# SoraSuegami/halo2-rsa

Measured on AMD Instinct MI355X. Metric: RSA-2048 pkcs1v15 witness assigns/sec, higher is better.
Workload: dtype u64

## Files before the change

halo2_rsa_amd/csrc/h2r_api.hip:

```cpp
#include <hip/hip_runtime.h>
#include <hip/hip_ext.h>
#include <dlfcn.h>
#include <rccl/rccl.h>

#include <algorithm>
#include <chrono>
#include <cstdio>
#include <cstdlib>
#include <cstring>
#include <functional>
#include <map>
#include <memory>
#include <mutex>
#include <new>
#include <vector>

#include "h2r.h"
#include "h2r_internal.hpp"
#include "h2r_varrows.hpp"
#include "h2r_copymap.hpp"
#include "h2r_layout.hpp"
#include "h2r_lookup.hpp"
#include "h2r_lookup_product.hpp"
#include "h2r_permutation_product.hpp"
#include "h2r_ntt.hpp"
#include "h2r_quotient.hpp"
#include "h2r_open.hpp"
#include "h2r_msm.hpp"
#include "h2r_curve_ntt.hpp"
#include "h2r_transcript.hpp"
#include "h2r_random.hpp"
#include "h2r_verify.hpp"
#include "h2r_muled.hpp"
#include "h2r_rowprog.hpp"
#include "h2r_sha256.hpp"
#include "h2r_check.hpp"
#include "h2r_arena_match.hpp"
#include "h2r_stage_args.hpp"

using namespace h2r;

namespace {

thread_local char g_hip_err[256] = "";

bool hip_ok(hipError_t e, const char *what) {
    if (e == hipSuccess) return true;
    std::snprintf(g_hip_err, sizeof g_hip_err, "%s: %s", what, hipGetErrorString(e));
    return false;
}
#define H2R_CATCH_STATUS catch (const std::bad_alloc &) { return H2R_E_NOMEM; } catch (...) { return H2R_E_INTERNAL; }
#define H2R_CATCH_ZERO catch (...) { return 0; }
#define H2R_CATCH_VOID catch (...) { }
#define H2R_CATCH_STR catch (...) { return ""; }
#define HIP_TRY(expr)                                   \
    do {                                                \
        if (!hip_ok((expr), #expr)) return H2R_E_HIP;   \
    } while (0)

struct DeviceGuard {
    int prev = -1; bool switched = false; hipError_t err = hipSuccess;
    explicit DeviceGuard(int dev) {
        err = hipGetDevice(&prev);
        if (err == hipSuccess && prev != dev) { err = hipSetDevice(dev); switched = err == hipSuccess; }
    }
    ~DeviceGuard() { if (switched) (void)hipSetDevice(prev); }
    DeviceGuard(const DeviceGuard &) = delete;
    DeviceGuard &operator=(const DeviceGuard &) = delete;
};
#define H2R_ON_DEVICE(dev_)                                     \
    DeviceGuard h2r_device_guard_(dev_);                        \
    if (!hip_ok(h2r_device_guard_.err, "hipSetDevice")) return H2R_E_HIP

struct ProfRec { u32 kernel; hipEvent_t a, b; };
std::mutex g_prof_mu;
std::vector<ProfRec> g_prof;
u32 g_prof_cap = 0;
u32 g_prof_gen = 0;
struct ProfScope {
    hipStream_t st; hipEvent_t a = nullptr, b = nullptr; u32 kernel; bool on = false, ext;
    ProfScope(u32 k, hipStream_t s, bool ext_ = false) : st(s), kernel(k), ext(ext_) {
        std::lock_guard<std::mutex> lk(g_prof_mu);
        if (g_prof_cap && g_prof.size() < g_prof_cap && hipEventCreate(&a) == hipSuccess) {
            if (hipEventCreate(&b) != hipSuccess) { (void)hipEventDestroy(a); a = nullptr; return; }
            on = true;
            if (!ext) (void)hipEventRecord(a, st);
        }
    }
    ~ProfScope() {
        if (!on) return;
        if (!ext) (void)hipEventRecord(b, st);
        std::lock_guard<std::mutex> lk(g_prof_mu);
        g_prof.push_back(ProfRec{kernel, a, b});
    }
};
template <class Fn> int32_t stage_launch(u32 kernel_class, hipStream_t st, Fn &&fn) {
    ProfScope ps(kernel_class, st, true);
    HIP_TRY(fn(ps.a, ps.on ? ps.b : nullptr));
    return H2R_OK;
}


inline u64 odd_stride_256(u64 bytes) {
    u64 u = round_up(bytes, 256) / 256;
    u |= 1;
    const u64 r = u % 256;
    if (r >= 24 && r <= 62) u += 65 - r;
    return u * 256;
}

struct DoneRef {
    hipEvent_t ev = nullptr; u32 gen = 0; bool borrowed = false;
    bool alive() const {
        if (!borrowed) return true;
        std::lock_guard<std::mutex> lk(g_prof_mu);
        return gen == g_prof_gen;
    }
};

struct Workspace {
    u64 off_pre;
    u64 off_n;
    u64 off_state;
    u64 total;
};
Workspace workspace_plan(u32 limb_bytes, u32 L, u64 batch, u32 T) {
    Workspace w;
    const u64 arr = round_up(batch * T * (u64)L * limb_bytes, 256);
    w.off_pre = 4 * arr;
    w.off_n = w.off_pre + round_up(4ull * chain_pre_words(128), 256);
    w.off_state = w.off_n + round_up(batch * (u64)L * limb_bytes, 256);
    w.total = w.off_state + round_up(2 * batch * (u64)L * limb_bytes, 256) + 256;
    return w;
}

}

struct h2r_ctx {
    h2r_params params;
    h2r_layout layout;
    u32 L, K;
    U256 word_max;
    u8 *const_rec_dev;
    u32 *advice_desc_dev = nullptr;
    u32 cells_nwv = 1;
    u64 *cells_ktab_dev = nullptr;
    std::vector<u8> const_rec_host;
    u32 tab0_len, tab1_off, tab1_len, tab2_off, tab2_len, hist_len;
    u8 refresh_inc[2 * 128 + 8]; u32 refresh_nf;
    u64 field_p[4];
    FieldConsts fc;
    h2r_advice_repr repr;
    MontK mk;
    MontK *mk_dev = nullptr;
    u32 num_cus, lds_per_cu;
    mutable std::mutex pipe_mu;
    mutable h2r_pipeline *pipe = nullptr;
    mutable std::mutex side_mu;
    mutable hipStream_t side_stream = nullptr;
    mutable hipEvent_t side_fork = nullptr, side_join = nullptr;
    struct RowProg { std::vector<RpRow> host; RpRow *dev = nullptr; std::vector<u32> inv_rows; u32 *inv_dev = nullptr; };
    mutable std::mutex prog_mu;
    mutable std::map<u32, RowProg> progs;
    mutable std::mutex check_mu;
    mutable std::map<std::vector<u8>, CheckKind *> check_tabs;
};

namespace {

void put_le(u8 *dst, const U256 &v, u32 nbytes) { std::memcpy(dst, v.v, nbytes); }

void build_const_record(h2r_ctx *c) {
    const h2r_layout &lo = c->layout;
    c->const_rec_host.assign(lo.record_stride, 0);
    u8 *r = c->const_rec_host.data();
    const u32 w = lo.limb_width, C = lo.num_cols;
    U256 acc_extra;
    for (u32 i = 0; i < C; ++i) {
        acc_extra = acc_extra + c->word_max;
        U256 q_acc = acc_extra.shr(w);
        u64 mod_acc = acc_extra.low(w);
// ... 2076 lines not shown
    return lookup_hist_values_impl(ctx, cfg, values, value_bytes, values_per_elem, num_elems, values_per_elem * value_bytes, value_bytes,
                                   bit_len, sublimb_bits, nullptr, hist, stream);
} H2R_CATCH_STATUS

int32_t h2r_lookup_hist_values_strided(const h2r_ctx *ctx, const h2r_lookup_config *cfg, const void *values, uint32_t value_bytes,
                                       uint64_t values_per_elem, uint64_t num_elems, uint64_t elem_stride, uint64_t value_stride,
                                       uint32_t bit_len, uint32_t sublimb_bits, const uint8_t *status, uint32_t *hist,
                                       h2r_stream_t stream) try {
    return lookup_hist_values_impl(ctx, cfg, values, value_bytes, values_per_elem, num_elems, elem_stride, value_stride, bit_len,
                                   sublimb_bits, status, hist, stream);
} H2R_CATCH_STATUS

extern "C++" {
namespace {
template <typename F>
void fresh_range_runs(const AuxGeom &g, u32 op, F &&run) {
    u64 off = 0;
    const u32 L = g.L;
    auto add = [&](u32 n) { run(off + 2 * g.SB, n, g.STEP); run(off + 2 * g.SB + g.RA, n, g.STEP); off += g.add_sz(n); };
    auto eq = [&](u32 n) { off += g.eq_sz(n); };
    auto subu = [&](u32 n1) { run(off, n1, g.RA); off += g.cl_sz(n1); add(n1); eq(n1 + 1); };
    auto sub = [&](u32 nA, u32 nB) {
        const u32 m = nA > nB ? nA : nB, n1 = m + 1;
        add(m); subu(n1);
        off += 16; off += AuxGeom::a16((u64)n1 * g.LB); off += AuxGeom::a16((u64)m * g.LB);
        subu(n1);
    };
    auto lt = [&]() { sub(L, L); eq(L); off += 16; };
    switch (op) {
        case FRESH_ADD: add(L); break;
        case FRESH_SUB: case FRESH_IS_LESS_THAN_OR_EQUAL: case FRESH_IS_GREATER_THAN: sub(L, L); break;
        case FRESH_ADD_MOD: add(L); sub(L + 1, L); break;
        case FRESH_SUB_MOD: sub(L, L); sub(L, L + 1); break;
        case FRESH_IS_LESS_THAN: case FRESH_IS_IN_FIELD: case FRESH_IS_GREATER_THAN_OR_EQUAL: lt(); break;
        default: break;
    }
}
int32_t lookup_hist_fresh_impl(const h2r_ctx *ctx, const h2r_lookup_config *cfg, uint32_t op, const void *trace, uint64_t first_off,
                               uint64_t elem_stride, uint64_t num_elems, const uint8_t *status, uint32_t *hist, h2r_stream_t stream) {
    if (!ctx || !cfg || !trace || !hist) return H2R_E_NULL;
    if (ctx->params.device < 0 || op >= FRESH_OP_COUNT) return H2R_E_UNSUPPORTED;
    if (cfg->n_rows == 0 || cfg->n_rows > (u32)LOOKUP_MAX_ROWS) return H2R_E_SHAPE;
    const h2r_layout &lo = ctx->layout;
    LookupFreshArgs a;
    std::memset(&a, 0, sizeof a);
    a.status = status;
    const int32_t rc = range_shape(*cfg, lo.limb_width, lo.limb_sub_bits, &a.limb);
    if (rc) return rc;
    const AuxGeom g(ctx->L, lo.limb_width);
    bool too_many = false;
    fresh_range_runs(g, op, [&](u64 off, u32 n, u32 stride) {
        if (a.n_runs >= 16) { too_many = true; return; }
        a.run_off[a.n_runs] = (u32)off; a.run_n[a.n_runs] = n; a.run_stride[a.n_runs] = stride; ++a.n_runs;
    });
    if (too_many) return H2R_E_UNSUPPORTED;
    if (num_elems == 0 || a.n_runs == 0) return H2R_OK;
    a.trace = static_cast<const u8 *>(trace); a.first_off = first_off; a.elem_stride = elem_stride; a.num_elems = num_elems;
    a.sub_off = lo.limb_bytes; a.n_rows = cfg->n_rows; a.hist = hist;
    H2R_ON_DEVICE(ctx->params.device);
    hipStream_t st = static_cast<hipStream_t>(stream);
    ProfScope ps(H2R_KERNEL_HIST, st);
    HIP_TRY(launch_lookup_hist_fresh(a, st));
    return H2R_OK;
}
}
}

int32_t h2r_lookup_hist_verify(const h2r_ctx *ctx, const h2r_lookup_config *cfg, const h2r_verify_layout *vl, const void *trace,
                               uint64_t num_elems, const uint8_t *status, uint32_t *hist, h2r_stream_t stream) try {
    if (!ctx || !cfg || !vl || !trace || !hist) return H2R_E_NULL;
    if (vl->pow.off_records == UINT64_MAX) return H2R_E_SHAPE;
    int32_t rc = lookup_hist_fresh_impl(ctx, cfg, H2R_OP_IS_IN_FIELD, trace, vl->off_in_field, vl->elem_stride, num_elems, status, hist, stream);
    if (!rc) rc = h2r_lookup_hist_records(ctx, cfg, trace, vl->pow.off_records, vl->elem_stride, num_elems, vl->pow.num_mul_mods, status, hist, stream);
    if (!rc) rc = lookup_hist_values_impl(ctx, cfg, static_cast<const u8 *>(trace) + vl->off_em + 12, 4, 2, num_elems, vl->elem_stride, 12, 32, 4,
                                          status, hist, stream);
    return rc;
} H2R_CATCH_STATUS

int32_t h2r_lookup_hist_fresh_op(const h2r_ctx *ctx, const h2r_lookup_config *cfg, uint32_t op, const void *trace, uint64_t first_off,
                                 uint64_t elem_stride, uint64_t num_elems, uint32_t *hist, h2r_stream_t stream) try {
    return lookup_hist_fresh_impl(ctx, cfg, op, trace, first_off, elem_stride, num_elems, nullptr, hist, stream);
} H2R_CATCH_STATUS

uint64_t h2r_lookup_workspace_bytes(const h2r_lookup_config *cfg, uint64_t num_elems) try {
    if (!cfg || cfg->n_rows == 0 || cfg->n_rows > (u32)LOOKUP_MAX_ROWS) return 0;
    return num_elems * LOOKUP_ARGS * lookup_slot_bytes(cfg->n_rows) + 256;
} H2R_CATCH_ZERO

int32_t h2r_lookup_permuted_columns(const h2r_ctx *ctx, const h2r_lookup_config *cfg, const uint32_t *hist, const uint64_t *theta,
                                    uint64_t num_elems, uint32_t usable_rows, uint32_t arg_mask, void *a_perm_out,
                                    void *s_perm_out, uint64_t out_elem_stride, uint8_t *status, void *workspace,
                                    h2r_stream_t stream) try {
    if (!ctx || !cfg || !hist || !theta || !a_perm_out || !s_perm_out || !workspace) return H2R_E_NULL;
    if (ctx->params.device < 0) return H2R_E_UNSUPPORTED;
    if (cfg->n_rows == 0 || cfg->n_rows > (u32)LOOKUP_MAX_ROWS || cfg->n_lens == 0 || cfg->n_lens > H2R_LOOKUP_MAX_LENS) return H2R_E_SHAPE;
    if (usable_rows < cfg->n_rows || out_elem_stride < (u64)LOOKUP_ARGS * usable_rows * 32 || (out_elem_stride & 15) ||
        (reinterpret_cast<u64>(a_perm_out) & 15) || (reinterpret_cast<u64>(s_perm_out) & 15)) return H2R_E_SHAPE;
    if (num_elems == 0 || !(arg_mask & 31u)) return H2R_OK;
    if (num_elems * LOOKUP_ARGS >= (1ull << 31) || num_elems > 65535) return H2R_E_UNSUPPORTED;
    H2R_ON_DEVICE(ctx->params.device);
    hipStream_t st = static_cast<hipStream_t>(stream);
    u8 *ws = reinterpret_cast<u8 *>(round_up(reinterpret_cast<u64>(workspace), 256));
    if (status) HIP_TRY(hipMemsetAsync(status, 0, num_elems, st));
    LookupSetupArgs sa;
    std::memset(&sa, 0, sizeof sa);
    sa.hist = hist; sa.theta = theta; sa.num_elems = num_elems; sa.usable_rows = usable_rows; sa.n_rows = cfg->n_rows;
    sa.n_lens = cfg->n_lens; sa.arg_mask = arg_mask & 31u;
    for (u32 i = 0; i < cfg->n_lens; ++i) { sa.tag[i] = cfg->tag[i]; sa.row_off[i] = cfg->row_off[i]; sa.bit_len[i] = cfg->bit_len[i]; }
    sa.f = ctx->fc; sa.ws = ws; sa.status = status;
    sa.mont = (ctx->repr.flags & H2R_ADVICE_MONTGOMERY) ? 1u : 0u;
    HIP_TRY(launch_lookup_setup(sa, st));
    LookupFillArgs fa;
    std::memset(&fa, 0, sizeof fa);
    fa.ws = ws; fa.num_elems = num_elems; fa.usable_rows = usable_rows; fa.n_rows = cfg->n_rows; fa.arg_mask = arg_mask & 31u;
    fa.rows_per_block = 256; fa.round_robin = 0; fa.status = status;
#ifdef H2R_DEV_KNOBS
    if ((arg_mask >> 8) & 0xffu) fa.rows_per_block = 256u * ((arg_mask >> 8) & 0xffu);
    fa.round_robin = (arg_mask >> 16) & 1u;
#endif
    fa.a_perm = static_cast<u8 *>(a_perm_out); fa.s_perm = static_cast<u8 *>(s_perm_out); fa.out_elem_stride = out_elem_stride;
    return stage_launch(H2R_KERNEL_LOOKUP, st, [&](hipEvent_t a, hipEvent_t b) { return launch_lookup_fill(fa, st, a, b); });
} H2R_CATCH_STATUS

int32_t h2r_field_eval(const h2r_ctx *ctx, uint32_t op, const uint64_t a[4], const uint64_t b[4], uint64_t out[4]) try {
    if (!ctx || !a || !out || (op < 3 && !b)) return H2R_E_NULL;
    Fe x, y = fe_zero(), r;
    for (int k = 0; k < 4; ++k) { x.v[k] = a[k]; if (b) y.v[k] = b[k]; }
    if (ge_p(x.v, ctx->fc.p) || (op < 3 && ge_p(y.v, ctx->fc.p))) return H2R_E_SHAPE;
    switch (op) {
        case 0: r = fe_add(x, y, ctx->fc.p); break;
        case 1: r = fe_sub(x, y, ctx->fc.p); break;
        case 2: r = fe_mul(x, y, ctx->fc); break;
        case 3: if (fe_is_zero(x)) return H2R_E_SHAPE; r = fe_inv(x, ctx->fc); break;
        case 4: if (fe_is_zero(x)) return H2R_E_SHAPE; r = fe_inv_fermat(x, ctx->fc); break;
        case 5: if (fe_is_zero(x)) return H2R_E_SHAPE; r = fe_inv_fast(x, ctx->fc); break;
        case 6: {
            u32 d[8], t[8]; int K = 1;
            for (int k = 0; k < 4; ++k) { d[2 * k] = (u32)x.v[k]; d[2 * k + 1] = (u32)(x.v[k] >> 32); }
            for (int k = 0; k < 8; ++k) if (d[k]) K = k + 1;
            switch (K) {
                case 1: { const u32 q[1] = {d[0]}; mont_short<1>(q, ctx->mk.bk[1], ctx->mk.p, ctx->mk.n0inv, t); break; }
                case 2: { const u32 q[2] = {d[0], d[1]}; mont_short<2>(q, ctx->mk.bk[2], ctx->mk.p, ctx->mk.n0inv, t); break; }
                case 3: { const u32 q[3] = {d[0], d[1], d[2]}; mont_short<3>(q, ctx->mk.bk[3], ctx->mk.p, ctx->mk.n0inv, t); break; }
                case 4: { const u32 q[4] = {d[0], d[1], d[2], d[3]}; mont_short<4>(q, ctx->mk.bk[4], ctx->mk.p, ctx->mk.n0inv, t); break; }
                case 5: { const u32 q[5] = {d[0], d[1], d[2], d[3], d[4]}; mont_short<5>(q, ctx->mk.bk[5], ctx->mk.p, ctx->mk.n0inv, t); break; }
                case 6: { const u32 q[6] = {d[0], d[1], d[2], d[3], d[4], d[5]}; mont_short<6>(q, ctx->mk.bk[6], ctx->mk.p, ctx->mk.n0inv, t); break; }
                case 7: { const u32 q[7] = {d[0], d[1], d[2], d[3], d[4], d[5], d[6]}; mont_short<7>(q, ctx->mk.bk[7], ctx->mk.p, ctx->mk.n0inv, t); break; }
                default: mont_short<8>(d, ctx->mk.bk[8], ctx->mk.p, ctx->mk.n0inv, t); break;
            }
            for (int k = 0; k < 4; ++k) r.v[k] = ((u64)t[2 * k + 1] << 32) | t[2 * k];
            break;
        }
        case 7: r = fe_from_mont(x, ctx->fc); break;
        case 8: r = fe_to_mont(x, ctx->fc); break;
        case 9: {
            u32 d[8], t[8]; int bits = 1;
            for (int k = 0; k < 4; ++k) { d[2 * k] = (u32)x.v[k]; d[2 * k + 1] = (u32)(x.v[k] >> 32); }
            for (int k = 0; k < 256; ++k) if ((d[k / 32] >> (k % 32)) & 1u) bits = k + 1;
            switch ((bits + 29) / 30) {
                case 1: mont_bits<30, 8>(d, ctx->mk, t); break;
                case 2: mont_bits<60, 8>(d, ctx->mk, t); break;
                case 3: mont_bits<90, 8>(d, ctx->mk, t); break;
                case 4: mont_bits<120, 8>(d, ctx->mk, t); break;
                case 5: mont_bits<150, 8>(d, ctx->mk, t); break;
                case 6: mont_bits<180, 8>(d, ctx->mk, t); break;
                case 7: mont_bits<210, 8>(d, ctx->mk, t); break;
                case 8: mont_bits<240, 8>(d, ctx->mk, t); break;
                default: mont_bits<256, 8>(d, ctx->mk, t); break;
            }
            for (int k = 0; k < 4; ++k) r.v[k] = ((u64)t[2 * k + 1] << 32) | t[2 * k];
            break;
        }
        default: return H2R_E_UNSUPPORTED;
    }
    for (int k = 0; k < 4; ++k) out[k] = r.v[k];
    return H2R_OK;
} H2R_CATCH_STATUS

namespace {
struct Out { u8 *p; };
inline void emit(Out &o, const u8 *src, u32 n) { std::memcpy(o.p, src, n); o.p += n; }
inline void emit_wide(Out &o, const h2r_layout &lo, const u8 *rec, int pl_lo, u64 idx) {
    emit(o, rec + lo.plane_off[pl_lo] + idx * 16, lo.wide_bytes < 16 ? lo.wide_bytes : 16);
    if (lo.wide_bytes > 16) emit(o, rec + lo.plane_off[pl_lo + 1] + idx * 8, lo.wide_bytes - 16);
}
inline void emit_acc(Out &o, const h2r_layout &lo, const u8 *rec, int pl_lo, u32 j, u32 im) {
    const u64 g = j / lo.acc_steps_per_group, st = j % lo.acc_steps_per_group;
    emit(o, rec + lo.plane_off[pl_lo] + g * lo.acc_lo_group_bytes + st * lo.acc_lo_row_bytes + (u64)im * 16, lo.wide_bytes < 16 ? lo.wide_bytes : 16);
    if (lo.wide_bytes > 16) emit(o, rec + lo.plane_off[pl_lo + 1] + (u64)(j >> 1) * lo.acc_hi_group_bytes + (u64)im * 16 + (j & 1) * 8, lo.wide_bytes - 16);
}
inline void emit_plane(Out &o, const h2r_layout &lo, const u8 *rec, int pl, u64 idx, u32 n) {
    emit(o, rec + lo.plane_off[pl] + idx * lo.plane_elem[pl], n);
}
}

static u8 *flatten_parts(const h2r_layout &lo, const u8 *rec, u8 *outp, u32 parts, const u64 *fp = nullptr) {
    const u32 L = lo.num_limbs, C = lo.num_cols;
    Out o{outp};
    if (parts & 1)
        for (int which = 0; which < 2; ++which)
            for (u32 k = 0; k < L; ++k) {
                emit_plane(o, lo, rec, which ? H2R_PL_R : H2R_PL_Q, k, lo.limb_bytes);
                emit_plane(o, lo, rec, which ? H2R_PL_R_SUB : H2R_PL_Q_SUB, k, lo.limb_nsub);
            }
// ... 459 lines not shown
int32_t fresh_row_prog(const h2r_ctx *ctx, uint32_t op, uint32_t flags, const h2r_ctx::RowProg **out) {
    if (op >= FRESH_OP_COUNT) return H2R_E_UNSUPPORTED;
    const bool assert_one = (flags & H2R_ADVICE_ASSERT_ONE) != 0;
    return row_prog(ctx, op | (assert_one ? 256u : 0u), [&](RowProgBuilder &rb) { return rb.build(op, assert_one); }, out);
}
int32_t launch_row_prog(const h2r_ctx *ctx, const h2r_ctx::RowProg *rp, RowProgArgs &ra, hipStream_t st) {
    ra.prog = rp->dev; ra.rows = (u32)rp->host.size(); ra.f = ctx->fc; ra.mk = ctx->mk_dev;
    ra.inv_rows = rp->inv_dev; ra.n_inv = (u32)rp->inv_rows.size();
    const long sr_k = knobs().rowprog_stage_rows;
    const u32 sr_env = (sr_k == 64 || sr_k == 128 || sr_k == 256) ? (u32)sr_k : 0u;
    const u32 sr = sr_env ? sr_env : ((ctx->repr.flags & H2R_ADVICE_MONTGOMERY) ? 64u : 256u);
    const u64 blocks = ra.batch * ((ra.rows + sr - 1) / sr);
    if (blocks == 0) return H2R_OK;
    if (blocks >= (1ull << 31)) return H2R_E_UNSUPPORTED;
    const u32 w = ctx->layout.limb_width;
    if (const int32_t rc = stage_launch(H2R_KERNEL_EMIT, st, [&](hipEvent_t a, hipEvent_t b) { return launch_rowprog_shape(w, sr, ra, (u32)blocks, st, a, b); })) return rc;
    if (ra.n_inv) {
        const u32 nt = sr == 64 ? 64u : 256u;
        const u64 ib = (ra.batch * ra.n_inv + nt - 1) / nt;
        if (ib >= (1ull << 31)) return H2R_E_UNSUPPORTED;
        HIP_TRY(launch_rowprog_inv_shape(w, nt, ra, (u32)ib, st));
    }
    return H2R_OK;
}
}

uint32_t h2r_fresh_op_advice_rows(const h2r_ctx *ctx, uint32_t op, uint32_t flags) try {
    const h2r_ctx::RowProg *rp = nullptr;
    if (!ctx || fresh_row_prog(ctx, op, flags, &rp)) return 0;
    return (uint32_t)rp->host.size();
} H2R_CATCH_ZERO

int32_t h2r_fresh_op_row_kinds(const h2r_ctx *ctx, uint32_t op, uint32_t flags, uint8_t *kinds_out) try {
    if (!ctx || !kinds_out) return H2R_E_NULL;
    const h2r_ctx::RowProg *rp = nullptr;
    const int32_t rc = fresh_row_prog(ctx, op, flags, &rp);
    if (rc) return rc;
    for (size_t r = 0; r < rp->host.size(); ++r) kinds_out[r] = (uint8_t)rp->host[r].kind;
    return H2R_OK;
} H2R_CATCH_STATUS

namespace {
int32_t fresh_emit_advice(const h2r_ctx *ctx, uint32_t op, uint32_t flags, const void *a, const void *b, const void *n,
                          const void *trace, uint64_t first_off, uint64_t elem_stride, uint64_t batch, const uint8_t *status,
                          const AdviceDst *dst_in, void *advice_out, uint64_t out_stride, h2r_stream_t stream) {
    if (!ctx || !a || !trace || (!dst_in && !advice_out)) return H2R_E_NULL;
    if (ctx->params.device < 0) return H2R_E_UNSUPPORTED;
    const h2r_ctx::RowProg *rp = nullptr;
    int32_t rc = fresh_row_prog(ctx, op, flags, &rp);
    if (rc) return rc;
    const bool needs_b = op != FRESH_IS_ZERO, needs_n = op == FRESH_ADD_MOD || op == FRESH_SUB_MOD;
    if ((needs_b && !b) || (needs_n && !n)) return H2R_E_NULL;
    u64 es = 0;
    rc = h2r_fresh_op_layout(ctx, op, &es, nullptr, nullptr);
    if (rc) return rc;
    if (elem_stride == 0) elem_stride = es;
    const u64 rows = rp->host.size();
    if ((first_off & 15) || (elem_stride & 15)) return H2R_E_SHAPE;
    AdviceDst dst;
    if (dst_in) dst = *dst_in;
    else if ((rc = advice_dst(ctx, advice_out, out_stride, rows, batch, &dst))) return rc;
    if (batch == 0) return H2R_OK;
    RowProgArgs ra;
    std::memset(&ra, 0, sizeof ra);
    ra.a = a; ra.b = b ? b : a; ra.n = n ? n : a;
    ra.a_stride = ctx->L;
    ra.n_stride = (flags & H2R_F_SHARED_MODULUS) ? 0 : ctx->L;
    ra.b_stride = (!needs_n && (flags & H2R_F_SHARED_MODULUS)) ? 0 : ctx->L;
    ra.trace = static_cast<const u8 *>(trace); ra.elem_stride = elem_stride; ra.first_off = first_off;
    ra.status = status; ra.batch = batch; ra.dst = dst;
    H2R_ON_DEVICE(ctx->params.device);
    return launch_row_prog(ctx, rp, ra, static_cast<hipStream_t>(stream));
}
}

int32_t h2r_fresh_op_emit_advice(const h2r_ctx *ctx, uint32_t op, uint32_t flags, const void *a, const void *b, const void *n,
                                 const void *trace, uint64_t first_off, uint64_t elem_stride, uint64_t batch, const uint8_t *status,
                                 void *advice_out, uint64_t out_stride, h2r_stream_t stream) try {
    if (const int32_t g = moduli_guard(flags, n, false)) return g;
    return fresh_emit_advice(ctx, op, flags, a, b, n, trace, first_off, elem_stride, batch, status, nullptr, advice_out, out_stride, stream);
} H2R_CATCH_STATUS

namespace {
struct SideFork {
    const h2r_ctx *ctx; hipStream_t main; std::unique_lock<std::mutex> lk; bool ok = false;
    SideFork(const h2r_ctx *c, hipStream_t st) : ctx(c), main(st), lk(c->side_mu) {
        hipStreamCaptureStatus cs = hipStreamCaptureStatusNone;
        if (hipStreamIsCapturing(main, &cs) != hipSuccess) { (void)hipGetLastError(); return; }
        if (cs != hipStreamCaptureStatusNone) return;
        if (!ctx->side_stream) {
            if (hipStreamCreateWithFlags(&ctx->side_stream, hipStreamNonBlocking) != hipSuccess ||
                hipEventCreateWithFlags(&ctx->side_fork, hipEventDisableTiming) != hipSuccess ||
                hipEventCreateWithFlags(&ctx->side_join, hipEventDisableTiming) != hipSuccess) { (void)hipGetLastError(); return; }
        }
        ok = hipEventRecord(ctx->side_fork, main) == hipSuccess && hipStreamWaitEvent(ctx->side_stream, ctx->side_fork, 0) == hipSuccess;
        if (!ok) (void)hipGetLastError();
    }
    hipStream_t side() const { return ok ? ctx->side_stream : main; }
    int32_t join() {
        if (!ok) return H2R_OK;
        ok = false;
        HIP_TRY(hipEventRecord(ctx->side_join, ctx->side_stream));
        HIP_TRY(hipStreamWaitEvent(main, ctx->side_join, 0));
        return H2R_OK;
    }
    ~SideFork() { if (ok) (void)join(); }
    SideFork(const SideFork &) = delete;
    SideFork &operator=(const SideFork &) = delete;
};

int32_t verify_progs(const h2r_ctx *ctx, const h2r_ctx::RowProg **pre, const h2r_ctx::RowProg **inf, const h2r_ctx::RowProg **em) {
    if (ctx->layout.limb_width != 64 || ctx->L < 8) return H2R_E_UNSUPPORTED;
    int32_t rc = row_prog(ctx, kProgVerifyPre, [](RowProgBuilder &rb) { rb.build_verify_preamble(); return true; }, pre);
    if (!rc) rc = fresh_row_prog(ctx, FRESH_IS_IN_FIELD, H2R_ADVICE_ASSERT_ONE, inf);
    if (!rc) rc = row_prog(ctx, kProgEm, [](RowProgBuilder &rb) { rb.build_em(); return true; }, em);
    return rc;
}
}

uint64_t h2r_verify_advice_rows(const h2r_ctx *ctx, const h2r_verify_layout *vl, uint64_t section_rows[4]) try {
    if (!ctx || !vl) return 0;
    const h2r_ctx::RowProg *pre, *inf, *em;
    if (verify_progs(ctx, &pre, &inf, &em)) return 0;
    const u64 r[4] = {pre->host.size(), inf->host.size(), h2r_pow_advice_rows(ctx, &vl->pow), em->host.size()};
    if (section_rows) for (int k = 0; k < 4; ++k) section_rows[k] = r[k];
    return r[0] + r[1] + r[2] + r[3];
} H2R_CATCH_ZERO

int32_t h2r_verify_row_kinds(const h2r_ctx *ctx, const h2r_verify_layout *vl, uint8_t *kinds_out) try {
    if (!ctx || !vl || !kinds_out) return H2R_E_NULL;
    const h2r_ctx::RowProg *pre, *inf, *em;
    const int32_t rc = verify_progs(ctx, &pre, &inf, &em);
    if (rc) return rc;
    uint8_t *k = kinds_out;
    for (const RpRow &r : pre->host) *k++ = (uint8_t)r.kind;
    for (const RpRow &r : inf->host) *k++ = (uint8_t)r.kind;
    if (int32_t rk = h2r_pow_row_kinds(ctx, &vl->pow, k)) return rk;
    k += h2r_pow_advice_rows(ctx, &vl->pow);
    for (const RpRow &r : em->host) *k++ = (uint8_t)r.kind;
    return H2R_OK;
} H2R_CATCH_STATUS

int32_t h2r_verify_emit_advice(const h2r_ctx *ctx, const h2r_verify_layout *vl, const void *sig, const void *n, const uint64_t *hashed,
                               const void *powed, uint32_t flags, const void *trace, const void *workspace, uint64_t batch,
                               const uint8_t *status, void *advice_out, uint64_t out_stride, h2r_stream_t stream) try {
    if (const int32_t g = moduli_guard(flags, n, false)) return g;
    if (!ctx || !vl || !sig || !n || !hashed || !powed || !trace || !workspace || !advice_out) return H2R_E_NULL;
    if (ctx->params.device < 0) return H2R_E_UNSUPPORTED;
    const h2r_ctx::RowProg *pre, *inf, *em;
    int32_t rc = verify_progs(ctx, &pre, &inf, &em);
    if (rc) return rc;
    u64 sec[4];
    const u64 rows = h2r_verify_advice_rows(ctx, vl, sec);
    AdviceDst dst;
    if ((rc = advice_dst(ctx, advice_out, out_stride, rows, batch, &dst))) return rc;
    if (batch == 0) return H2R_OK;
    H2R_ON_DEVICE(ctx->params.device);
    hipStream_t st = static_cast<hipStream_t>(stream);
    SideFork fork(ctx, st);
    hipStream_t ss = fork.side();
    RowProgArgs ra;
    std::memset(&ra, 0, sizeof ra);
    ra.a = sig; ra.b = n; ra.n = n; ra.a_stride = ctx->L; ra.b_stride = ra.n_stride = (flags & H2R_F_SHARED_MODULUS) ? 0 : ctx->L;
    ra.trace = static_cast<const u8 *>(trace); ra.elem_stride = vl->elem_stride; ra.first_off = vl->off_in_field;
    ra.status = status; ra.batch = batch;
    ra.dst = dst;
    if ((rc = launch_row_prog(ctx, pre, ra, ss))) return rc;
    ra.dst = dst.at_row(sec[0]);
    if ((rc = launch_row_prog(ctx, inf, ra, ss))) return rc;
    ra.a = powed; ra.b = hashed; ra.b_stride = 4; ra.first_off = vl->off_em;
    ra.dst = dst.at_row(sec[0] + sec[1] + sec[2]);
    if ((rc = launch_row_prog(ctx, em, ra, ss))) return rc;
    rc = pow_emit_advice(ctx, &vl->pow, n, flags, trace, vl->elem_stride, workspace, batch, status,
                         dst.at_row(sec[0] + sec[1]), stream);
    if (rc) return rc;
    return fork.join();
} H2R_CATCH_STATUS

uint32_t h2r_advice_copy_map(const h2r_ctx *ctx, h2r_copy *out, uint32_t cap) try {
    if (!ctx) return 0;
    std::vector<h2r_copy> v;
    copy_map_record(ctx->L, (ctx->layout.carry_nsub + 3) / 4, v);
    for (u32 i = 0; out && i < cap && i < v.size(); ++i) out[i] = v[i];
    return (uint32_t)v.size();
} H2R_CATCH_ZERO

int32_t h2r_pow_operand_sources(const h2r_ctx *ctx, const h2r_pow_layout *pl, const uint8_t *e_le_bytes, size_t e_len, int32_t *a_src, int32_t *b_src) try {
    if (!ctx || !pl || !a_src || !b_src) return H2R_E_NULL;
    if (pl->off_e_bits != UINT64_MAX) return H2R_E_UNSUPPORTED;
    ExpBits eb; u32 T;
    const int32_t rc = exp_to_bits(e_le_bytes, e_len, &eb, &T);
    if (rc) return rc;
    if (T != pl->num_mul_mods) return H2R_E_SHAPE;
// ... 2050 lines not shown
```

halo2_rsa_amd/csrc/h2r_lookup.hpp:

```cpp
#pragma once

#include "h2r_field.hpp"
#include "h2r_kernels.hpp"

namespace h2r {

constexpr int LOOKUP_ARGS = 5;
constexpr int LOOKUP_MAX_ROWS = 1024;
constexpr int LOOKUP_MAX_LENS = 8;

struct RangeShape {
    u32 nsub, sub_bits, ov_bits;
    u32 row_comp, row_ov;
};
__host__ __device__ inline u32 range_last_row(const RangeShape &s) { return (s.nsub - 1) / 4; }

template <typename SubFn>
__device__ __forceinline__ void range_count(u32 *h, u32 n_rows, const RangeShape &s, SubFn sub) {
    const u32 last = range_last_row(s), last_len = s.nsub - 4 * last;
    for (u32 t = 0; t < s.nsub; ++t) {
        const u32 v = sub(t);
        const u32 rr = t / 4;
        const u32 arg = rr < last ? (t & 3u) : (s.nsub - 1 - t);
        atomicAdd(&h[arg * n_rows + s.row_comp + v], 1u);
// ... 23 lines not shown
    for (u64 idx = tid; idx < (u64)a.records_per_elem * per_rec; idx += 256) {
        const u32 t = (u32)(idx / per_rec), k = (u32)(idx - (u64)t * per_rec);
        const u8 *rec = base + (u64)t * a.record_stride;
        if (k < 2 * a.L) {
            const u64 sb = *reinterpret_cast<const u64 *>(rec + (k < a.L ? a.off_q_sub + (u64)k * 8 : a.off_r_sub + (u64)(k - a.L) * 8));
            range_count(lh, a.n_rows, a.limb, [&](u32 i) { return (u32)((sb >> (8 * i)) & 0xff); });
        } else {
            const ulonglong2 sb = *reinterpret_cast<const ulonglong2 *>(rec + a.off_carry_sub + (u64)(k - 2 * a.L) * a.carry_sub_stride);
            range_count(lh, a.n_rows, a.carry, [&](u32 i) { return (u32)(((i < 8 ? sb.x : sb.y) >> (8 * (i & 7))) & 0xff); });
        }
    }
    __syncthreads();
    u32 *out = a.hist + elem * n;
    for (u32 k = tid; k < n; k += 256) if (lh[k]) out[k] += lh[k];
}
#endif

struct LookupValuesArgs {
    const u8 *values; u32 value_bytes; u64 values_per_elem, num_elems;
    u64 elem_stride, value_stride;
    const u8 *status;
    RangeShape shape; u32 n_rows; u32 *hist;
};
#ifdef H2R_TU_LOOKUP
__global__ __launch_bounds__(256) void lookup_hist_values_kernel(LookupValuesArgs a) {
    extern __shared__ u32 lh[];
    const u32 tid = threadIdx.x, n = LOOKUP_ARGS * a.n_rows;
    const u64 elem = blockIdx.x;
    if (a.status && a.status[elem]) return;
    for (u32 k = tid; k < n; k += 256) lh[k] = 0;
    __syncthreads();
    const u32 m = (1u << a.shape.sub_bits) - 1;
    for (u64 idx = tid; idx < a.values_per_elem; idx += 256) {
        const u8 *p = a.values + elem * a.elem_stride + idx * a.value_stride;
        u128 v = a.value_bytes == 4 ? (u128) * reinterpret_cast<const u32 *>(p) : (u128) * reinterpret_cast<const u64 *>(p);
        if (a.value_bytes == 16) v |= (u128)(*reinterpret_cast<const u64 *>(p + 8)) << 64;
        range_count(lh, a.n_rows, a.shape, [&](u32 i) { return (u32)(v >> (i * a.shape.sub_bits)) & m; });
    }
    __syncthreads();
    u32 *out = a.hist + elem * n;
    for (u32 k = tid; k < n; k += 256) if (lh[k]) out[k] += lh[k];
}
#endif

struct LookupFreshArgs {
    const u8 *trace; u64 first_off, elem_stride, num_elems;
    u32 n_runs; u32 run_off[16], run_n[16], run_stride[16]; u32 sub_off;
    RangeShape limb; u32 n_rows; u32 *hist; const u8 *status;
};
#ifdef H2R_TU_LOOKUP
__global__ __launch_bounds__(64) void lookup_hist_fresh_kernel(LookupFreshArgs a) {
    extern __shared__ u32 lh[];
    const u32 tid = threadIdx.x, n = LOOKUP_ARGS * a.n_rows;
    const u64 elem = blockIdx.x;
    if (a.status && a.status[elem]) return;
    for (u32 k = tid; k < n; k += 64) lh[k] = 0;
    __syncthreads();
    const u8 *base = a.trace + elem * a.elem_stride + a.first_off;
    for (u32 r = 0; r < a.n_runs; ++r)
        for (u32 i = tid; i < a.run_n[r]; i += 64) {
            const u8 *p = base + a.run_off[r] + (u64)i * a.run_stride[r] + a.sub_off;
            const u64 sb = (u64) * reinterpret_cast<const u32 *>(p) | ((u64) * reinterpret_cast<const u32 *>(p + 4) << 32);
            range_count(lh, a.n_rows, a.limb, [&](u32 t) { return (u32)((sb >> (8 * t)) & 0xff); });
        }
    __syncthreads();
    u32 *out = a.hist + elem * n;
    for (u32 k = tid; k < n; k += 64) if (lh[k]) out[k] += lh[k];
}
#endif

__host__ __device__ inline u64 lookup_slot_bytes(u32 n_rows) { return (u64)n_rows * 32 + ((u64)(3 * n_rows + 2 + 2) * 4 + 15) / 16 * 16; }

struct LookupSetupArgs {
    const u32 *hist;
    const u64 *theta;
    u32 mont;
    u64 num_elems; u32 usable_rows, n_rows, n_lens, arg_mask;
    u32 tag[LOOKUP_MAX_LENS], row_off[LOOKUP_MAX_LENS], bit_len[LOOKUP_MAX_LENS];
    FieldConsts f;
    u8 *ws;
    u8 *status;
};

__device__ __forceinline__ void block_scan_1024(u32 *x, u32 n, u32 *part ) {
    const u32 tid = threadIdx.x;
    const u32 per = (n + 255) / 256, lo = tid * per;
    u32 s = 0;
    for (u32 k = lo; k < lo + per && k < n; ++k) { s += x[k]; x[k] = s; }
    part[tid] = s;
    __syncthreads();
    for (u32 d = 1; d < 256; d <<= 1) {
        const u32 v = tid >= d ? part[tid - d] : 0;
        __syncthreads();
        part[tid] += v;
        __syncthreads();
    }
    const u32 add = tid ? part[tid - 1] : 0;
    for (u32 k = lo; k < lo + per && k < n; ++k) x[k] += add;
    __syncthreads();
}

__host__ __device__ inline u32 lookup_setup_lds_bytes(u32 n) { return n * 32u + LOOKUP_MAX_LENS * 32u + 5u * n * 4u + 256u * 4u + 16u; }
#ifdef H2R_TU_LOOKUP
__global__ __launch_bounds__(256) void lookup_setup_kernel(LookupSetupArgs a) {
    extern __shared__ uint4 ls_dyn[];
    const u32 tid = threadIdx.x, n = a.n_rows;
    Fe *T = reinterpret_cast<Fe *>(ls_dyn);
    Fe *tagth = T + n;
    u32 *order = reinterpret_cast<u32 *>(tagth + LOOKUP_MAX_LENS);
    u32 *gid = order + n;
    u32 *gm = gid + n, *gs = gm + n, *gr = gs + n;
    u32 *part = gr + n;
    u32 &total_in = part[256], &too_many = part[257];
    const u32 arg = blockIdx.x % LOOKUP_ARGS;
    const u64 elem = blockIdx.x / LOOKUP_ARGS;
    if (!((a.arg_mask >> arg) & 1u)) return;
    const u32 *h = a.hist + (elem * LOOKUP_ARGS + arg) * n;
    Fe theta;
    for (int k = 0; k < 4; ++k) theta.v[k] = a.theta[elem * 4 + k];
    const bool theta_ok = !ge_p(theta.v, a.f.p);
    if (a.mont && theta_ok) theta = fe_from_mont(theta, a.f);
    if (tid < a.n_lens) tagth[tid] = fe_mul_small(theta, a.tag[tid], a.f.p);
    if (tid == 0) { total_in = 0; too_many = 0; }
    __syncthreads();
    u64 my_in = 0;
    for (u32 r = tid; r < n; r += 256) {
        Fe t = fe_zero();
        if (r) {
            u32 i = 0;
            while (i + 1 < a.n_lens && r >= a.row_off[i + 1]) ++i;
            t = fe_add(tagth[i], fe_small(r - a.row_off[i]), a.f.p);
        }
        T[r] = t;
        my_in += h[r];
    }
    const u32 usable = a.usable_rows;
    if (my_in > usable) too_many = 1;
    else if (my_in) { const u32 before = atomicAdd(&total_in, (u32)my_in); if (before + (u32)my_in < before) too_many = 1; }
    __syncthreads();
    const bool fits = !too_many && total_in <= usable && n <= usable && theta_ok;
    if (!fits) {
        if (tid == 0) {
            if (a.status) a.status[elem] = (u8)H2R_E_SHAPE;
            u32 *gc = reinterpret_cast<u32 *>(a.ws + (elem * LOOKUP_ARGS + arg) * lookup_slot_bytes(n) + (u64)n * 32) + (3 * n + 2);
            gc[0] = 0; gc[1] = 0;
        }
        return;
    }
    for (u32 r = tid; r < n; r += 256) {
        const Fe me = T[r];
        u32 rank = r ? 1u : 0u;
        for (u32 j = 0; j < a.n_lens; ++j) {
            const Fe B = tagth[j];
            const u32 S = 1u << a.bit_len[j];
            auto small = [](const Fe &x, u32 cap) -> u32 { return ((x.v[1] | x.v[2] | x.v[3]) == 0 && x.v[0] < cap) ? (u32)x.v[0] : cap; };
            const Fe d = fe_sub(me, B, a.f.p);
            const bool ge = !fe_lt(me, B);
            Fe pm; for (int k = 0; k < 4; ++k) pm.v[k] = a.f.p[k];
            const Fe wj = fe_is_zero(B) ? pm : fe_sub(fe_zero(), B, a.f.p);
            const u32 W = small(wj, S);
            u32 less = ge ? small(d, W) : 0u;
            if (W < S) less += small(me, S - W);
            const u32 eq_u = small(d, S);
            if (eq_u < S && a.row_off[j] + eq_u < r) ++less;
            rank += less;
        }
        order[rank] = r;
    }
    __syncthreads();
    for (u32 i = tid; i < n; i += 256) gid[i] = (i == 0 || !fe_eq(T[order[i]], T[order[i - 1]])) ? 1u : 0u;
    for (u32 i = tid; i < n; i += 256) { gm[i] = 0; gs[i] = 0; }
    __syncthreads();
    block_scan_1024(gid, n, part);
    const u32 G = gid[n - 1];
    for (u32 i = tid; i < n; i += 256) {
        const u32 r = order[i], g = gid[i] - 1;
        const u32 m = h[r] + (r == 0 ? usable - total_in : 0u), s = 1u + (r == 0 ? usable - n : 0u);
        if (m) atomicAdd(&gm[g], m);
        atomicAdd(&gs[g], s);
    }
    __syncthreads();
    u8 *slot = a.ws + (elem * LOOKUP_ARGS + arg) * lookup_slot_bytes(n);
    Fe *val = reinterpret_cast<Fe *>(slot);
    u32 *a_start = reinterpret_cast<u32 *>(slot + (u64)n * 32), *a_rank = a_start + n + 1, *l_start = a_rank + n, *gcount = l_start + n + 1;
    for (u32 i = tid; i < n; i += 256) if (i == 0 || gid[i] != gid[i - 1]) val[gid[i] - 1] = a.mont ? fe_to_mont(T[order[i]], a.f) : T[order[i]];
    for (u32 g = tid; g < G; g += 256) { gr[g] = gm[g] ? 1u : 0u; gs[g] -= gr[g]; }
    __syncthreads();
    block_scan_1024(gm, G, part);
    block_scan_1024(gr, G, part);
    block_scan_1024(gs, G, part);
    for (u32 g = tid; g < G; g += 256) { a_start[g + 1] = gm[g]; a_rank[g] = g ? gr[g - 1] : 0u; l_start[g + 1] = gs[g]; }
    if (tid == 0) { a_start[0] = 0; l_start[0] = 0; gcount[0] = G; gcount[1] = gr[G - 1]; }
}
#endif

struct LookupFillArgs {
    const u8 *ws; u64 num_elems; u32 usable_rows, n_rows, arg_mask, rows_per_block, round_robin;
    const u8 *status;
    u8 *a_perm, *s_perm; u64 out_elem_stride;
};
__device__ __forceinline__ u32 upper_group(const u32 *start, u32 G, u32 x) {
    u32 lo = 0, hi = G;
    while (lo < hi) { const u32 mid = (lo + hi + 1) >> 1; if (start[mid] <= x) lo = mid; else hi = mid - 1; }
    return lo;
}
#ifdef H2R_TU_LOOKUP
__global__ __launch_bounds__(256) void lookup_fill_kernel(LookupFillArgs a) {
    extern __shared__ uint4 lf_dyn[];
    const u32 tid = threadIdx.x, lane = tid & 63, n = a.n_rows;
    const u32 chunk = blockIdx.x, arg = blockIdx.y;
    const u64 elem = blockIdx.z;
    if (!((a.arg_mask >> arg) & 1u)) return;
    if (a.status && a.status[elem]) return;
    const u64 slot_bytes = lookup_slot_bytes(n);
    const uint4 *src = reinterpret_cast<const uint4 *>(a.ws + (elem * LOOKUP_ARGS + arg) * slot_bytes);
    for (u32 k = tid; k < slot_bytes / 16; k += 256) lf_dyn[k] = src[k];
    __syncthreads();
    const u8 *slot = reinterpret_cast<const u8 *>(lf_dyn);
    const Fe *val = reinterpret_cast<const Fe *>(slot);
    const u32 *a_start = reinterpret_cast<const u32 *>(slot + (u64)n * 32), *a_rank = a_start + n + 1, *l_start = a_rank + n, *gcount = l_start + n + 1;
    const u32 G = gcount[0], n_heads = gcount[1];
    if (G == 0) return;
    const u32 usable = a.usable_rows, n_rep = usable - n_heads;
    u8 *ap = a.a_perm + elem * a.out_elem_stride + (u64)arg * usable * 32;
    u8 *sp = a.s_perm + elem * a.out_elem_stride + (u64)arg * usable * 32;
    const bool rr = a.round_robin != 0;
    const u32 p0 = rr ? chunk * 256 : chunk * a.rows_per_block;
    const u32 p1 = rr ? usable : (p0 + a.rows_per_block < usable ? p0 + a.rows_per_block : usable);
    const u32 base_step = rr ? 256 * gridDim.x : 256;
    for (u32 base = p0 + (tid & ~63u); base < p1; base += base_step) {
        const u32 pos = base + lane;
        Fe av = fe_zero(), sv = fe_zero();
        if (pos < p1) {
            const u32 g = upper_group(a_start, G, pos);
            av = val[g];
            if (pos == a_start[g]) sv = av;
            else {
                const u32 j = pos - (a_rank[g] + 1);
                const u32 li = n_rep - 1 - j;
                sv = val[upper_group(l_start, G, li)];
            }
        }
#pragma unroll
        for (int hlf = 0; hlf < 2; ++hlf) {
            const int srcl = 32 * hlf + (int)(lane >> 1);
            const bool hi = lane & 1;
            const u64 a0 = __shfl(av.v[0], srcl), a1 = __shfl(av.v[1], srcl), a2 = __shfl(av.v[2], srcl), a3 = __shfl(av.v[3], srcl);
            const u64 s0 = __shfl(sv.v[0], srcl), s1 = __shfl(sv.v[1], srcl), s2 = __shfl(sv.v[2], srcl), s3 = __shfl(sv.v[3], srcl);
            const u32 row = base + 32 * hlf + (lane >> 1);
            if (row < p1) {
                st16(ap + (u64)row * 32 + (hi ? 16 : 0), hi ? a2 : a0, hi ? a3 : a1);
                st16(sp + (u64)row * 32 + (hi ? 16 : 0), hi ? s2 : s0, hi ? s3 : s1);
            }
        }
    }
}
#endif

}
```

Before: 6.156 million.

## Slice lookup permuted-column launches and overlap setup with fill on side stream

Removes the hard num_elems limit on lookup permuted-column generation by splitting work into slices bounded by a launch limit. When several slices are needed, the setup kernel for the next slice runs on a side stream while the fill kernel for the current slice runs on the main stream. The block scan is rewritten to use wave shuffles and to scan three arrays in one pass, and histogram counts are cached in shared memory rather than re-read. With FIRST_SLICE=0 and large limits, usually only one slice runs, so the overlap may rarely trigger.

```diff
diff --git a/halo2_rsa_amd/csrc/h2r_api.hip b/halo2_rsa_amd/csrc/h2r_api.hip
--- a/halo2_rsa_amd/csrc/h2r_api.hip
+++ b/halo2_rsa_amd/csrc/h2r_api.hip
@@ -36,6 +36,7 @@
 #include "h2r_sha256.hpp"
 #include "h2r_check.hpp"
 #include "h2r_arena_match.hpp"
+#include "h2r_lookup_slices.hpp"
 #include "h2r_stage_args.hpp"
 
 using namespace h2r;
@@ -97,6 +98,12 @@
 template <class Fn> int32_t stage_launch(u32 kernel_class, hipStream_t st, Fn &&fn) {
     ProfScope ps(kernel_class, st, true);
     HIP_TRY(fn(ps.a, ps.on ? ps.b : nullptr));
+    return H2R_OK;
+}
+
+template <class Fn> int32_t stage_span(u32 kernel_class, hipStream_t st, u64 n, Fn &&fn) {
+    ProfScope ps(kernel_class, st, true);
+    for (u64 i = 0; i < n; ++i) HIP_TRY(fn(i, i == 0 ? ps.a : nullptr, ps.on && i + 1 == n ? ps.b : nullptr));
     return H2R_OK;
 }
 
@@ -2339,6 +2346,42 @@
     return lookup_hist_fresh_impl(ctx, cfg, op, trace, first_off, elem_stride, num_elems, nullptr, hist, stream);
 } H2R_CATCH_STATUS
 
+namespace {
+struct SideFork {
+    const h2r_ctx *ctx; hipStream_t main; std::unique_lock<std::mutex> lk; bool ok = false;
+    SideFork(const h2r_ctx *c, hipStream_t st) : ctx(c), main(st), lk(c->side_mu) {
+        hipStreamCaptureStatus cs = hipStreamCaptureStatusNone;
+        if (hipStreamIsCapturing(main, &cs) != hipSuccess) { (void)hipGetLastError(); return; }
+        if (cs != hipStreamCaptureStatusNone) return;
+        if (!ctx->side_stream) {
+            if (hipStreamCreateWithFlags(&ctx->side_stream, hipStreamNonBlocking) != hipSuccess ||
+                hipEventCreateWithFlags(&ctx->side_fork, hipEventDisableTiming) != hipSuccess ||
+                hipEventCreateWithFlags(&ctx->side_join, hipEventDisableTiming) != hipSuccess) { (void)hipGetLastError(); return; }
+        }
+        ok = hipEventRecord(ctx->side_fork, main) == hipSuccess && hipStreamWaitEvent(ctx->side_stream, ctx->side_fork, 0) == hipSuccess;
+        if (!ok) (void)hipGetLastError();
+    }
+    hipStream_t side() const { return ok ? ctx->side_stream : main; }
+    int32_t join() {
+        if (!ok) return H2R_OK;
+        ok = false;
+        HIP_TRY(hipEventRecord(ctx->side_join, ctx->side_stream));
+        HIP_TRY(hipStreamWaitEvent(main, ctx->side_join, 0));
+        return H2R_OK;
+    }
+    int32_t main_waits() {
+        if (!ok) return H2R_OK;
+        HIP_TRY(hipEventRecord(ctx->side_join, ctx->side_stream));
+        HIP_TRY(hipStreamWaitEvent(main, ctx->side_join, 0));
+        return H2R_OK;
+    }
+    void close() { ok = false; }
+    ~SideFork() { if (ok) (void)join(); }
+    SideFork(const SideFork &) = delete;
+    SideFork &operator=(const SideFork &) = delete;
+};
+}
+
 uint64_t h2r_lookup_workspace_bytes(const h2r_lookup_config *cfg, uint64_t num_elems) try {
     if (!cfg || cfg->n_rows == 0 || cfg->n_rows > (u32)LOOKUP_MAX_ROWS) return 0;
     return num_elems * LOOKUP_ARGS * lookup_slot_bytes(cfg->n_rows) + 256;
@@ -2354,29 +2397,57 @@
     if (usable_rows < cfg->n_rows || out_elem_stride < (u64)LOOKUP_ARGS * usable_rows * 32 || (out_elem_stride & 15) ||
         (reinterpret_cast<u64>(a_perm_out) & 15) || (reinterpret_cast<u64>(s_perm_out) & 15)) return H2R_E_SHAPE;
     if (num_elems == 0 || !(arg_mask & 31u)) return H2R_OK;
-    if (num_elems * LOOKUP_ARGS >= (1ull << 31) || num_elems > 65535) return H2R_E_UNSUPPORTED;
+    LookupFillArgs fa;
+    std::memset(&fa, 0, sizeof fa);
+    fa.usable_rows = usable_rows; fa.n_rows = cfg->n_rows; fa.arg_mask = arg_mask & 31u;
+    fa.rows_per_block = 256; fa.round_robin = 0;
+    u64 first = h2r_lookup_slices::FIRST_SLICE;
+#ifdef H2R_DEV_KNOBS
+    if ((arg_mask >> 8) & 0xffu) fa.rows_per_block = 256u * ((arg_mask >> 8) & 0xffu);
+    fa.round_robin = (arg_mask >> 16) & 1u;
+    if ((arg_mask >> 17) & 0xffu) first = ((arg_mask >> 17) & 0xffu) == 255u ? 0 : (arg_mask >> 17) & 0xffu;
+#endif
+    fa.out_elem_stride = out_elem_stride;
+    const u64 chunks = (usable_rows + fa.rows_per_block - 1) / fa.rows_per_block;
+    const u64 limit = h2r_lookup_slices::launch_limit(chunks * LOOKUP_ARGS);
+    if (!limit) return H2R_E_UNSUPPORTED;
     H2R_ON_DEVICE(ctx->params.device);
     hipStream_t st = static_cast<hipStream_t>(stream);
     u8 *ws = reinterpret_cast<u8 *>(round_up(reinterpret_cast<u64>(workspace), 256));
     if (status) HIP_TRY(hipMemsetAsync(status, 0, num_elems, st));
     LookupSetupArgs sa;
     std::memset(&sa, 0, sizeof sa);
-    sa.hist = hist; sa.theta = theta; sa.num_elems = num_elems; sa.usable_rows = usable_rows; sa.n_rows = cfg->n_rows;
-    sa.n_lens = cfg->n_lens; sa.arg_mask = arg_mask & 31u;
+    sa.usable_rows = usable_rows; sa.n_rows = cfg->n_rows; sa.n_lens = cfg->n_lens; sa.arg_mask = arg_mask & 31u;
     for (u32 i = 0; i < cfg->n_lens; ++i) { sa.tag[i] = cfg->tag[i]; sa.row_off[i] = cfg->row_off[i]; sa.bit_len[i] = cfg->bit_len[i]; }
-    sa.f = ctx->fc; sa.ws = ws; sa.status = status;
+    sa.f = ctx->fc;
     sa.mont = (ctx->repr.flags & H2R_ADVICE_MONTGOMERY) ? 1u : 0u;
-    HIP_TRY(launch_lookup_setup(sa, st));
-    LookupFillArgs fa;
-    std::memset(&fa, 0, sizeof fa);
-    fa.ws = ws; fa.num_elems = num_elems; fa.usable_rows = usable_rows; fa.n_rows = cfg->n_rows; fa.arg_mask = arg_mask & 31u;
-    fa.rows_per_block = 256; fa.round_robin = 0; fa.status = status;
-#ifdef H2R_DEV_KNOBS
-    if ((arg_mask >> 8) & 0xffu) fa.rows_per_block = 256u * ((arg_mask >> 8) & 0xffu);
-    fa.round_robin = (arg_mask >> 16) & 1u;
-#endif
-    fa.a_perm = static_cast<u8 *>(a_perm_out); fa.s_perm = static_cast<u8 *>(s_perm_out); fa.out_elem_stride = out_elem_stride;
-    return stage_launch(H2R_KERNEL_LOOKUP, st, [&](hipEvent_t a, hipEvent_t b) { return launch_lookup_fill(fa, st, a, b); });
+    const u64 slot5 = LOOKUP_ARGS * lookup_slot_bytes(cfg->n_rows);
+    auto setup = [&](const h2r_lookup_slices::Slice &sl, hipStream_t on) {
+        sa.hist = hist + sl.lo * LOOKUP_ARGS * cfg->n_rows; sa.theta = theta + sl.lo * 4; sa.num_elems = sl.count;
+        sa.ws = ws + sl.lo * slot5; sa.status = status ? status + sl.lo : nullptr;
+        return launch_lookup_setup(sa, on);
+    };
+    auto fill = [&](const h2r_lookup_slices::Slice &sl, hipEvent_t a, hipEvent_t b) {
+        fa.ws = ws + sl.lo * slot5; fa.num_elems = sl.count; fa.status = status ? status + sl.lo : nullptr;
+        fa.a_perm = static_cast<u8 *>(a_perm_out) + sl.lo * out_elem_stride; fa.s_perm = static_cast<u8 *>(s_perm_out) + sl.lo * out_elem_stride;
+        return launch_lookup_fill(fa, st, a, b);
+    };
+    h2r_lookup_slices::Plan plan(num_elems, first, limit);
+    const u64 ns = plan.count();
+    if (ns == 1) {
+        HIP_TRY(setup(plan.at(0), st));
+        return stage_launch(H2R_KERNEL_LOOKUP, st, [&](hipEvent_t a, hipEvent_t b) { return fill(plan.at(0), a, b); });
+    }
+    SideFork sf(ctx, st);
+    HIP_TRY(setup(plan.at(0), st));
+    const int32_t rc = stage_span(H2R_KERNEL_LOOKUP, st, ns, [&](u64 i, hipEvent_t a, hipEvent_t b) {
+        hipError_t e = fill(plan.at(i), a, b);
+        if (e != hipSuccess || i + 1 == ns) return e;
+        if ((e = setup(plan.at(i + 1), sf.side())) != hipSuccess) return e;
+        return sf.main_waits() == H2R_OK ? hipSuccess : hipErrorUnknown;
+    });
+    if (rc == H2R_OK) sf.close();
+    return rc;
 } H2R_CATCH_STATUS
 
 int32_t h2r_field_eval(const h2r_ctx *ctx, uint32_t op, const uint64_t a[4], const uint64_t b[4], uint64_t out[4]) try {
@@ -3002,33 +3073,6 @@
 } H2R_CATCH_STATUS
 
 namespace {
-struct SideFork {
-    const h2r_ctx *ctx; hipStream_t main; std::unique_lock<std::mutex> lk; bool ok = false;
-    SideFork(const h2r_ctx *c, hipStream_t st) : ctx(c), main(st), lk(c->side_mu) {
-        hipStreamCaptureStatus cs = hipStreamCaptureStatusNone;
-        if (hipStreamIsCapturing(main, &cs) != hipSuccess) { (void)hipGetLastError(); return; }
-        if (cs != hipStreamCaptureStatusNone) return;
-        if (!ctx->side_stream) {
-            if (hipStreamCreateWithFlags(&ctx->side_stream, hipStreamNonBlocking) != hipSuccess ||
-                hipEventCreateWithFlags(&ctx->side_fork, hipEventDisableTiming) != hipSuccess ||
-                hipEventCreateWithFlags(&ctx->side_join, hipEventDisableTiming) != hipSuccess) { (void)hipGetLastError(); return; }
-        }
-        ok = hipEventRecord(ctx->side_fork, main) == hipSuccess && hipStreamWaitEvent(ctx->side_stream, ctx->side_fork, 0) == hipSuccess;
-        if (!ok) (void)hipGetLastError();
-    }
-    hipStream_t side() const { return ok ? ctx->side_stream : main; }
-    int32_t join() {
-        if (!ok) return H2R_OK;
-        ok = false;
-        HIP_TRY(hipEventRecord(ctx->side_join, ctx->side_stream));
-        HIP_TRY(hipStreamWaitEvent(main, ctx->side_join, 0));
-        return H2R_OK;
-    }
-    ~SideFork() { if (ok) (void)join(); }
-    SideFork(const SideFork &) = delete;
-    SideFork &operator=(const SideFork &) = delete;
-};
-
 int32_t verify_progs(const h2r_ctx *ctx, const h2r_ctx::RowProg **pre, const h2r_ctx::RowProg **inf, const h2r_ctx::RowProg **em) {
     if (ctx->layout.limb_width != 64 || ctx->L < 8) return H2R_E_UNSUPPORTED;
     int32_t rc = row_prog(ctx, kProgVerifyPre, [](RowProgBuilder &rb) { rb.build_verify_preamble(); return true; }, pre);
diff --git a/halo2_rsa_amd/csrc/h2r_lookup.hpp b/halo2_rsa_amd/csrc/h2r_lookup.hpp
--- a/halo2_rsa_amd/csrc/h2r_lookup.hpp
+++ b/halo2_rsa_amd/csrc/h2r_lookup.hpp
@@ -129,21 +129,32 @@
     u8 *status;
 };
 
-__device__ __forceinline__ void block_scan_1024(u32 *x, u32 n, u32 *part ) {
-    const u32 tid = threadIdx.x;
+template <int K>
+__device__ __forceinline__ void block_scan_1024(u32 *const (&x)[K], u32 n, u32 *part ) {
+    const u32 tid = threadIdx.x, lane = tid & 63u, wave = tid >> 6;
     const u32 per = (n + 255) / 256, lo = tid * per;
-    u32 s = 0;
-    for (u32 k = lo; k < lo + per && k < n; ++k) { s += x[k]; x[k] = s; }
-    part[tid] = s;
-    __syncthreads();
-    for (u32 d = 1; d < 256; d <<= 1) {
-        const u32 v = tid >= d ? part[tid - d] : 0;
-        __syncthreads();
-        part[tid] += v;
-        __syncthreads();
-    }
-    const u32 add = tid ? part[tid - 1] : 0;
-    for (u32 k = lo; k < lo + per && k < n; ++k) x[k] += add;
+    u32 own[K], incl[K];
+#pragma unroll
+    for (int k = 0; k < K; ++k) {
+        u32 s = 0;
+        for (u32 i = lo; i < lo + per && i < n; ++i) { s += x[k][i]; x[k][i] = s; }
+        own[k] = incl[k] = s;
+    }
+    for (u32 d = 1; d < 64; d <<= 1) {
+#pragma unroll
+        for (int k = 0; k < K; ++k) { const u32 v = __shfl_up(incl[k], d); if (lane >= d) incl[k] += v; }
+    }
+    if (lane == 63) {
+#pragma unroll
+        for (int k = 0; k < K; ++k) part[4 * k + wave] = incl[k];
+    }
+    __syncthreads();
+#pragma unroll
+    for (int k = 0; k < K; ++k) {
+        u32 add = incl[k] - own[k];
+        for (u32 w = 0; w < wave; ++w) add += part[4 * k + w];
+        for (u32 i = lo; i < lo + per && i < n; ++i) x[k][i] += add;
+    }
     __syncthreads();
 }
 
@@ -179,7 +190,9 @@
             t = fe_add(tagth[i], fe_small(r - a.row_off[i]), a.f.p);
         }
         T[r] = t;
-        my_in += h[r];
+        const u32 c = h[r];
+        gr[r] = c;
+        my_in += c;
     }
     const u32 usable = a.usable_rows;
     if (my_in > usable) too_many = 1;
@@ -218,11 +231,11 @@
     for (u32 i = tid; i < n; i += 256) gid[i] = (i == 0 || !fe_eq(T[order[i]], T[order[i - 1]])) ? 1u : 0u;
     for (u32 i = tid; i < n; i += 256) { gm[i] = 0; gs[i] = 0; }
     __syncthreads();
-    block_scan_1024(gid, n, part);
+    { u32 *const one[1] = {gid}; block_scan_1024(one, n, part); }
     const u32 G = gid[n - 1];
     for (u32 i = tid; i < n; i += 256) {
         const u32 r = order[i], g = gid[i] - 1;
-        const u32 m = h[r] + (r == 0 ? usable - total_in : 0u), s = 1u + (r == 0 ? usable - n : 0u);
+        const u32 m = gr[r] + (r == 0 ? usable - total_in : 0u), s = 1u + (r == 0 ? usable - n : 0u);
         if (m) atomicAdd(&gm[g], m);
         atomicAdd(&gs[g], s);
     }
@@ -233,9 +246,7 @@
     for (u32 i = tid; i < n; i += 256) if (i == 0 || gid[i] != gid[i - 1]) val[gid[i] - 1] = a.mont ? fe_to_mont(T[order[i]], a.f) : T[order[i]];
     for (u32 g = tid; g < G; g += 256) { gr[g] = gm[g] ? 1u : 0u; gs[g] -= gr[g]; }
     __syncthreads();
-    block_scan_1024(gm, G, part);
-    block_scan_1024(gr, G, part);
-    block_scan_1024(gs, G, part);
+    { u32 *const three[3] = {gm, gr, gs}; block_scan_1024(three, G, part); }
     for (u32 g = tid; g < G; g += 256) { a_start[g + 1] = gm[g]; a_rank[g] = g ? gr[g - 1] : 0u; l_start[g + 1] = gs[g]; }
     if (tid == 0) { a_start[0] = 0; l_start[0] = 0; gcount[0] = G; gcount[1] = gr[G - 1]; }
 }
diff --git a/halo2_rsa_amd/csrc/h2r_lookup_slices.hpp b/halo2_rsa_amd/csrc/h2r_lookup_slices.hpp
--- /dev/null
+++ b/halo2_rsa_amd/csrc/h2r_lookup_slices.hpp
@@ -0,0 +1,29 @@
+#pragma once
+#include <cstdint>
+
+#include "h2r_stage_args.hpp"
+
+namespace h2r_lookup_slices {
+
+constexpr uint64_t FIRST_SLICE = 0;
+
+inline uint64_t launch_limit(uint64_t fill_workgroups_per_circuit) {
+    return fill_workgroups_per_circuit ? h2r_stage_args::slice_items(fill_workgroups_per_circuit, ~0ull) : 0;
+}
+
+struct Slice { uint64_t lo, count; };
+
+struct Plan {
+    uint64_t n = 0, head = 0, limit = 0;
+    Plan(uint64_t num_elems, uint64_t first, uint64_t limit_) : n(limit_ ? num_elems : 0), limit(limit_) {
+        if (first && n > first) head = first < limit ? first : limit;
+    }
+    uint64_t count() const { return n ? (head ? 1 : 0) + (n - head + limit - 1) / limit : 0; }
+    Slice at(uint64_t i) const {
+        if (head && i == 0) return Slice{0, head};
+        const uint64_t lo = head + (i - (head ? 1 : 0)) * limit;
+        return Slice{lo, n - lo < limit ? n - lo : limit};
+    }
+};
+
+}
```

Result: no change. 6.164 million, median of 5 (+0.1%).
